# HpWang-whu/RoReg

Measured on AMD Instinct MI355X. Metric: pair-registrations/sec, higher is better.
Workload: dtype f32 (every f32 operand enters the fp16 matrix cores as hi + lo fp16 under a per-keypoint power-of-two block scale: <= 22 significant bits relative to a CONSERVATIVE per-keypoint bound -- measured on the extractor: the bound sits 2^2..2^6 above the keypoint's true coefficient maximum (config.f16x2_sc

## Files before the change

include/roreg_hip.h:

```cpp
#ifndef ROREG_HIP_H
#define ROREG_HIP_H

#include <stdint.h>
#include <stddef.h>

#ifdef __cplusplus
extern "C" {
#endif

#define ROREG_ABI_VERSION 6
int roreg_abi_version(void);
const char *roreg_last_error(void);

int roreg_set_group_tables(const int32_t *P_host, const int32_t *Nei_host, const double *R_host);

size_t roreg_group_conv_packed_size(int Cin, int Cout, int KS);
int roreg_group_conv_pack_weights(const float *W_host , int Cin, int Cout, int KS,
                                  float *wpack_host );
size_t roreg_group_conv_workspace_size(int B, int Cin, int Cout, int Lin, int Lout, int KS);
int roreg_group_conv(const float *x, const float *wpack, const float *bias,
                     const float *bn_scale, const float *bn_shift, const float *residual,
                     float *out, const int32_t *gather,
                     int B, int Cin, int Cout, int Lin, int Lout, int KS,
                     float *workspace, size_t workspace_floats, void *stream);
// ... 174 lines not shown
int roreg_context_colmax(const float *R, int L, const int32_t *seg_off, int n_seg, int max_len, float *ctx_out, float *ws, void *stream);

int roreg_knn_attention(const float *qp, const float *kp, const float *vp, const int64_t *idx, int k_is_table, int v_is_table,
                        int m, int k, float *x_out, void *stream);

int roreg_rm_elementwise(int op, const float *a, const float *b, const float *c, const int64_t *idx, int L, int k, int C,
                         float *out, float *ws, void *stream);

size_t roreg_sinkhorn_workspace_size(int m, int n);
int roreg_sinkhorn(const float *src_final, int m, const float *tgt_final, int n, float alpha, int iters, float *Z_out,
                   int64_t *matches0, int64_t *matches1, float *mscores0, float *mscores1, float *ws, size_t ws_floats, void *stream);

size_t roreg_sinkhorn_batch_workspace_size(int n_seg, int max_m, int max_n, long long total_m, long long total_n);
int roreg_sinkhorn_batch_consts(const int32_t *seg_src_host, const int32_t *seg_tgt_host, int n_seg, float *consts_host);
int roreg_sinkhorn_batch(const float *src_final, const float *tgt_final, const int32_t *seg_src, const int32_t *seg_tgt,
                         const int32_t *seg_src_host, const int32_t *seg_tgt_host, const float *consts, int n_seg, float alpha, int iters,
                         int64_t *matches0, int64_t *matches1, float *mscores0, float *mscores1, float *ws, size_t ws_floats,
                         void *stream);

size_t roreg_sinkhorn_batch2_workspace_size(int n_seg, int max_m, int max_n, long long total_m, long long total_n);
int roreg_sinkhorn_batch2(const float *src_final, const float *tgt_final, const int32_t *seg_src, const int32_t *seg_tgt,
                          const int32_t *seg_src_host, const int32_t *seg_tgt_host, const float *consts, int n_seg, float alpha, int iters,
                          int64_t *matches0, int64_t *matches1, float *mscores0, float *mscores1, float *ws, size_t ws_floats,
                          int recompute, void *stream);
size_t roreg_sinkhorn_batch3_workspace_size(int n_seg, int max_m, int max_n, long long total_m, long long total_n, int recompute, int want_Z);
int roreg_sinkhorn_batch3(const float *src_final, const float *tgt_final, const int32_t *seg_src, const int32_t *seg_tgt,
                          const int32_t *seg_src_host, const int32_t *seg_tgt_host, const float *consts, int n_seg, float alpha, int iters,
                          int64_t *matches0, int64_t *matches1, float *mscores0, float *mscores1, float *ws, size_t ws_floats,
                          int recompute, float *Z_out, void *stream);
int roreg_write_files(const char *const *paths, const void *const *headers, const int32_t *header_len, const void *const *data,
                      const int64_t *nbytes, int n, int n_threads);
int roreg_yohoc_draw_many(const uint32_t *seeds, int n_pairs, const int64_t *anchors, const int64_t *offsets, int max_iter, int max_tries,
                          int64_t *rows_out, int32_t *n_hyp_out, double *giveup_out, int n_threads);
size_t roreg_mlp_head_workspace(int L, int n_seg, int C1);
int roreg_mlp_head(const float *x, const float *pos, const float *table, const int64_t *idx, const float *conf, int m, int k, int L, int Cin,
                   const float *W1, const float *b1, int C1, const float *Wr, const float *br, float *h, float *y, const int32_t *seg_off,
                   int n_seg, int mult, float eps, float *mean_rstd, double *ws, void *stream);
int roreg_sinkhorn_early_exit(int on);
int roreg_sinkhorn_iteration_stats(long long *iterations, long long *pairs, int reset, void *stream);

int roreg_set_fourier_tables(const float *F_host);
size_t roreg_irrep_gemm_tiles(int O, int B, int32_t *tiles_host);
size_t roreg_irrep_gemm_tiles_m(int O, int B, int tile_m , int32_t *tiles_host);
int roreg_irrep_gemm(const float *const *X, float *const *Out, const float *const *Add, const float *const *Wpack, int C, int O, int B,
                     const int32_t *tiles_dev, int n_tiles, void *stream);
int roreg_irrep_gemm_split(const float *const *X, float *const *Out, const float *const *Add, const void *const *Wsplit, int C, int O, int B,
                           const int32_t *tiles_dev, int n_tiles, void *stream);
int roreg_irrep_gemm_f16x2(const float *const *X, float *const *Out, const float *const *Add, const void *const *Wsplit2,
                           const float *x_bound_dev, int w_exp, const float *next_u_dev, const float *next_v_dev, float *out_bound_dev,
                           int C, int O, int B, const int32_t *tiles_dev, int n_tiles,
                           int tile_m ,
                           int x_planes , void *stream);
int roreg_gemm_persistent(int on);
int roreg_row_bound(const void *x_spatial, int x_bf16 , const float *bn_scale, const float *bn_shift,
                    float *bound_out, int B, int C, void *stream);
int roreg_ft_nonlin(const float *Xin , const float *x_spatial, const float *bias,
                    const float *bias2, const float *bn_scale, const float *bn_shift, const float *resid_spatial,
                    float *Xout , float *out_spatial ,
                    const int32_t *g_map ,
                    int Lout , int Lvalid,
                    int B, int C, int split ,
                    const float *out_bound ,
                    float *out_rowmax ,
                    int spatial_bf16 ,
                    int out_planes ,
                    void *stream);
int roreg_ft_nonlin_packed(const float *Xin, const float *bias, const float *bn_scale, const float *bn_shift, uint32_t *out_words,
                           const int32_t *g_map, int Lout, int Lvalid, int B, int C, const float *out_bound, float *raw_col, int raw_g,
                           void *stream);
int roreg_ft_nonlin_gathered(const uint64_t *rows , const int64_t *dr , int feat_bf16, const float *bn_scale ,
                             const float *bn_shift, float *Xout, int B, const float *out_bound , int out_planes, void *stream);

typedef struct roreg_icp_grid_desc {
    double origin[3];
    double edge;
    int32_t dims[3];
    int32_t n;
    int64_t cells;
    int64_t reserved;
} roreg_icp_grid_desc;
size_t roreg_icp_grid_size(const double *lo_host, const double *hi_host, int n, double max_dist, roreg_icp_grid_desc *desc_host,
                           size_t *workspace_bytes);
int roreg_icp_grid_build(const float *points, const roreg_icp_grid_desc *desc_host, void *grid, void *workspace, size_t workspace_bytes,
                         void *stream);
typedef struct roreg_icp_task {
    const void *tgt_grid;
    const void *src_grid;
    const double *T0;
    int32_t n_src;
    int32_t slot0;
} roreg_icp_task;
size_t roreg_icp_batch_workspace(int n_tasks, long long total_slots);
int roreg_icp_batch(const roreg_icp_task *tasks, int n_tasks, const int32_t *work, int n_work, long long total_slots, double max_dist,
                    int max_iter, double tol_deg, double tol_t, double *T_out, int32_t *iters_out, int32_t *inliers_out, double *rmse_out,
                    int32_t *status_out, int32_t *assign_out, double *stats_out, void *workspace, size_t workspace_bytes, void *stream);

int roreg_icp_normals(const void *grid, double radius, int min_neighbors, double *out, void *stream);
typedef struct roreg_icp_plane_task {
    const void *tgt_grid;
    const void *src_grid;
    const double *tgt_normals;
    const double *T0;
    int32_t n_src;
    int32_t slot0;
} roreg_icp_plane_task;
size_t roreg_icp_plane_batch_workspace(int n_tasks, long long total_slots);
// ... 16 lines not shown
```

roreg_amd/_abi.py:

```python
import ctypes
from ctypes import c_int, c_void_p, c_size_t, c_double, c_float, c_char_p

import numpy as np

ABI_VERSION = 6

_P = c_void_p
PROTOTYPES = {
    'roreg_abi_version': (c_int, []),
    'roreg_last_error': (c_char_p, []),
    'roreg_set_group_tables': (c_int, [_P, _P, _P]),
    'roreg_group_conv_packed_size': (c_size_t, [c_int, c_int, c_int]),
    'roreg_group_conv_pack_weights': (c_int, [_P, c_int, c_int, c_int, _P]),
    'roreg_group_conv_workspace_size': (c_size_t, [c_int, c_int, c_int, c_int, c_int, c_int]),
    'roreg_group_conv': (c_int, [_P, _P, _P, _P, _P, _P, _P, _P, c_int, c_int, c_int, c_int, c_int, c_int, _P, c_size_t, _P]),
    'roreg_group_conv_split': (c_int, [_P, _P, _P, _P, _P, _P, _P, _P, c_int, c_int, c_int, c_int, c_int, c_int, c_int, _P]),
    'roreg_group_conv_f16x2': (c_int, [_P, _P, c_int, _P, _P, _P, c_float, c_float, _P, _P, _P, _P, _P, c_int, c_int, c_int, c_int, c_int, c_int, c_int, _P]),
    'roreg_group_conv_f16x2_packed': (c_int, [_P, _P, c_int, _P, _P, _P, _P, _P, _P, c_int, c_int, c_int, c_int, c_int, c_int, c_int, _P]),
    'roreg_dense_f16x2': (c_int, [_P, _P, c_int, _P, _P, _P, c_float, c_float, _P, _P, c_int, _P, _P, c_int, c_int, c_int, _P]),
    'roreg_dense_split': (c_int, [_P, _P, _P, _P, _P, _P, c_int, _P, c_int, c_int, c_int, _P]),
    'roreg_gf_finalize': (c_int, [_P, _P, c_int, _P, c_int, _P]),
    'roreg_det_score': (c_int, [_P, _P, c_int, _P]),
    'roreg_inv_descriptor': (c_int, [_P, c_int, _P, c_int, _P]),
    'roreg_nn_search': (c_int, [_P, _P, c_int, _P, _P, c_int, c_int, _P, _P, _P, _P]),
# ... 2 lines not shown
    'roreg_knn_search_workspace': (c_size_t, [c_int, c_int]),
    'roreg_knn_search': (c_int, [_P, c_int, _P, c_int, c_int, c_int, _P, _P, c_size_t, _P]),
    'roreg_knn_search_ex': (c_int, [_P, c_int, _P, c_int, c_int, c_int, c_int, _P, _P, _P, c_size_t, _P]),
    'roreg_knn_search_seg_workspace': (c_size_t, [ctypes.c_longlong, c_int, c_int, c_int]),
    'roreg_knn_search_seg': (c_int, [_P, _P, _P, _P, c_int, ctypes.c_longlong, c_int, c_int, c_int, c_int, _P, _P, c_size_t, _P]),
    'roreg_mutual_matches': (c_int, [_P, _P, c_int, c_int, _P, _P, _P, _P, _P]),
    'roreg_mutual_match_batch_workspace': (c_size_t, [c_int, c_int]),
    'roreg_mutual_match_batch': (c_int, [_P, c_int, c_int, _P, _P, _P, c_size_t, _P]),
    'roreg_des2r': (c_int, [_P, _P, _P, _P, c_int, _P, _P, _P]),
    'roreg_set_des2r_tables': (c_int, [c_int, _P, _P, _P, _P]),
    'roreg_group_corr_irrep': (c_int, [_P, _P, _P, _P, c_int, c_int, _P, _P]),
    'roreg_group_corr_mfma': (c_int, [_P, _P, _P, _P, c_int, c_int, _P, _P]),
    'roreg_des2r_irrep': (c_int, [_P, _P, _P, _P, _P, _P, c_int, c_int, _P, _P]),
    'roreg_des2r_recheck_count': (c_int, [c_int, _P]),
    'roreg_feat_coefs': (c_int, [_P, c_int, _P, c_int, c_int, c_int, _P]),
    'roreg_et_gather': (c_int, [_P, _P, _P, _P, c_int, _P, _P, _P, c_int, _P, _P]),
    'roreg_quat_to_trans': (c_int, [_P, _P, _P, _P, _P, _P, c_int, _P, _P, _P]),
    'roreg_ransac_score': (c_int, [_P, _P, _P, c_int, c_int, _P, _P, c_int, c_double, _P, _P, _P, _P]),
    'roreg_refine': (c_int, [_P, _P, _P, c_int, c_int, _P, c_int, _P, _P, _P, c_double, _P, _P, _P]),
    'roreg_lt_prepare_batch': (c_int, [_P, c_int, c_int, c_int, _P, _P, _P, _P, _P, _P]),
    'roreg_lt_finish_batch': (c_int, [_P, c_int, c_int, _P, _P, _P, _P]),
    'roreg_role_max': (c_int, [_P, _P, c_int, _P, _P, _P, c_int, _P]),
    'roreg_row_bound_roles': (c_int, [_P, c_int, _P, _P, _P, _P, c_int, _P]),
    'roreg_inv_descriptor_roles': (c_int, [_P, c_int, _P, _P, _P, _P, c_int, _P]),
    'roreg_lt_prepare_rows': (c_int, [_P, _P, c_int, c_int, c_int, _P, _P, _P, _P]),
    'roreg_ransac_batch_workspace': (c_size_t, [c_int, ctypes.c_longlong, c_int]),
    'roreg_ransac_batch': (c_int, [_P, c_int, ctypes.c_longlong, c_int, c_int, c_double, c_int, _P, _P, _P, _P, _P, _P, c_size_t, _P]),
    'roreg_refine_batch': (c_int, [_P, _P, c_int, ctypes.c_longlong, _P, ctypes.c_double, c_int, _P, _P, _P, _P]),
    'roreg_yohoc_draw': (c_int, [_P, ctypes.c_longlong, _P, _P, c_int, c_int, _P, _P, _P, _P]),
    'roreg_gather_rows_batch': (c_int, [_P, c_int, c_int, c_int, _P]),
    'roreg_gather_rows_f64': (c_int, [_P, _P, c_int, c_int, _P, _P]),
    'roreg_group_corr': (c_int, [_P, _P, _P, _P, c_int, c_int, _P, _P, _P]),
    'roreg_topk_dot_workspace_size': (c_size_t, [c_int, c_int, c_int]),
    'roreg_topk_dot': (c_int, [_P, c_int, _P, c_int, c_int, _P, _P, _P, c_size_t, _P, _P, c_int, c_int, c_int, _P]),
    'roreg_context_colmax': (c_int, [_P, c_int, _P, c_int, c_int, _P, _P, _P]),
    'roreg_sinkhorn_batch_workspace_size': (c_size_t, [c_int, c_int, c_int, ctypes.c_longlong, ctypes.c_longlong]),
    'roreg_sinkhorn_batch_consts': (c_int, [_P, _P, c_int, _P]),
    'roreg_sinkhorn_batch': (c_int, [_P, _P, _P, _P, _P, _P, _P, c_int, c_float, c_int, _P, _P, _P, _P, _P, c_size_t, _P]),
    'roreg_sinkhorn_batch2_workspace_size': (c_size_t, [c_int, c_int, c_int, ctypes.c_longlong, ctypes.c_longlong]),
    'roreg_sinkhorn_batch2': (c_int, [_P, _P, _P, _P, _P, _P, _P, c_int, c_float, c_int, _P, _P, _P, _P, _P, c_size_t, c_int, _P]),
    'roreg_sinkhorn_batch3_workspace_size': (c_size_t, [c_int, c_int, c_int, ctypes.c_longlong, ctypes.c_longlong, c_int, c_int]),
    'roreg_sinkhorn_batch3': (c_int, [_P, _P, _P, _P, _P, _P, _P, c_int, c_float, c_int, _P, _P, _P, _P, _P, c_size_t, c_int, _P, _P]),
    'roreg_write_files': (c_int, [_P, _P, _P, _P, _P, c_int, c_int]),
    'roreg_yohoc_draw_many': (c_int, [_P, c_int, _P, _P, c_int, c_int, _P, _P, _P, c_int]),
    'roreg_mlp_head_workspace': (c_size_t, [c_int, c_int, c_int]),
    'roreg_mlp_head': (c_int, [_P, _P, _P, _P, _P, c_int, c_int, c_int, c_int, _P, _P, c_int, _P, _P, _P, _P, _P, c_int, c_int, c_float, _P, _P, _P]),
    'roreg_sinkhorn_early_exit': (c_int, [c_int]),
    'roreg_sinkhorn_iteration_stats': (c_int, [_P, _P, c_int, _P]),
    'roreg_linear': (c_int, [_P, c_int, c_int, _P, _P, c_int, _P, _P]),
    'roreg_linear_mfma': (c_int, [_P, c_int, c_int, _P, _P, c_int, _P, _P]),
    'roreg_linear_path': (c_int, [c_int]),
    'roreg_linear_cat3': (c_int, [_P, _P, _P, _P, c_int, c_int, _P, _P, c_int, _P, _P]),
    'roreg_gemm_persistent': (c_int, [c_int]),
    'roreg_instnorm_stats': (c_int, [_P, c_int, c_int, c_float, _P, _P, _P, c_int, c_int, _P]),
    'roreg_mlp_tail': (c_int, [_P, c_int, c_int, _P, _P, _P, _P, _P, c_int, c_int, _P]),
    'roreg_mlp_tail_mfma': (c_int, [_P, c_int, c_int, _P, _P, _P, _P, _P, c_int, c_int, _P]),
    'roreg_knn_attention': (c_int, [_P, _P, _P, _P, c_int, c_int, c_int, c_int, _P, _P]),
    'roreg_rm_elementwise': (c_int, [c_int, _P, _P, _P, _P, c_int, c_int, c_int, _P, _P, _P]),
    'roreg_sinkhorn_workspace_size': (c_size_t, [c_int, c_int]),
    'roreg_sinkhorn': (c_int, [_P, c_int, _P, c_int, c_float, c_int, _P, _P, _P, _P, _P, _P, c_size_t, _P]),
    'roreg_icp_grid_size': (c_size_t, [_P, _P, c_int, c_double, _P, _P]),
    'roreg_icp_grid_build': (c_int, [_P, _P, _P, _P, c_size_t, _P]),
    'roreg_icp_batch_workspace': (c_size_t, [c_int, ctypes.c_longlong]),
    'roreg_icp_batch': (c_int, [_P, c_int, _P, c_int, ctypes.c_longlong, c_double, c_int, c_double, c_double, _P, _P, _P, _P, _P, _P, _P, _P, c_size_t, _P]),
    'roreg_icp_normals': (c_int, [_P, c_double, c_int, _P, _P]),
    'roreg_icp_plane_batch_workspace': (c_size_t, [c_int, ctypes.c_longlong]),
    'roreg_icp_plane_batch': (c_int, [_P, c_int, _P, c_int, ctypes.c_longlong, c_double, c_int, c_double, c_double, _P, _P, _P, _P, _P, _P, _P, _P, c_size_t, _P]),
    'roreg_voxel_workspace': (c_size_t, [c_int]),
    'roreg_voxel_downsample': (c_int, [_P, c_int, c_double, _P, _P, _P, _P, _P, _P, _P, c_size_t, _P]),
    'roreg_profile_enable': (c_int, [c_int]),
    'roreg_profile_read': (c_int, [c_int, _P, _P]),
    'roreg_set_fourier_tables': (c_int, [_P]),
    'roreg_mt_shuffle_prefix': (c_int, [_P, c_int, _P, c_int, c_int, _P, c_int]),
    'roreg_mt_stream_shuffle_prefix': (c_int, [_P, _P, _P, c_int, c_int, _P]),
    'roreg_irrep_gemm_tiles': (c_size_t, [c_int, c_int, _P]),
    'roreg_irrep_gemm_tiles_m': (c_size_t, [c_int, c_int, c_int, _P]),
    'roreg_irrep_gemm': (c_int, [_P, _P, _P, _P, c_int, c_int, c_int, _P, c_int, _P]),
    'roreg_irrep_gemm_split': (c_int, [_P, _P, _P, _P, c_int, c_int, c_int, _P, c_int, _P]),
    'roreg_irrep_gemm_f16x2': (c_int, [_P, _P, _P, _P, _P, c_int, _P, _P, _P, c_int, c_int, c_int, _P, c_int, c_int, c_int, _P]),
    'roreg_row_bound': (c_int, [_P, c_int, _P, _P, _P, c_int, c_int, _P]),
    'roreg_ft_nonlin': (c_int, [_P, _P, _P, _P, _P, _P, _P, _P, _P, _P, c_int, c_int, c_int, c_int, c_int, _P, _P, c_int, c_int, _P]),
    'roreg_ft_nonlin_packed': (c_int, [_P, _P, _P, _P, _P, _P, c_int, c_int, c_int, c_int, _P, _P, c_int, _P]),
    'roreg_ft_nonlin_gathered': (c_int, [_P, _P, c_int, _P, _P, _P, c_int, _P, c_int, _P]),
}


_RANSAC_TASK = np.dtype([('keys0', np.uint64), ('keys1', np.uint64), ('matches', np.uint64), ('w', np.uint64), ('Trans', np.uint64),
                         ('hyp_rows', np.uint64), ('M', np.int32), ('H', np.int32), ('koff', np.int64)])

_MATCH_TASK = np.dtype([('desc0', np.uint64), ('desc1', np.uint64), ('rows0', np.uint64), ('rows1', np.uint64), ('m0', np.int32), ('m1', np.int32)])

_GATHER_TASK = np.dtype([('src', np.uint64), ('rows', np.uint64), ('dst', np.uint64), ('n', np.int32), ('pad', np.int32)])

_LT_TASK = np.dtype([('before0', np.uint64), ('before1', np.uint64), ('after0', np.uint64), ('after1', np.uint64), ('keys0', np.uint64),
                     ('keys1', np.uint64), ('matches', np.uint64), ('sel', np.uint64), ('n', np.int32), ('pad', np.int32), ('off', np.int64),
                     ('coef0', np.uint64), ('coef1', np.uint64)])

_ICP_GRID_DESC = np.dtype([('origin', np.float64, 3), ('edge', np.float64), ('dims', np.int32, 3), ('n', np.int32), ('cells', np.int64),
                           ('reserved', np.int64)])

_ICP_TASK = np.dtype([('tgt_grid', np.uint64), ('src_grid', np.uint64), ('T0', np.uint64), ('n_src', np.int32), ('slot0', np.int32)])

_ICP_PLANE_TASK = np.dtype([('tgt_grid', np.uint64), ('src_grid', np.uint64), ('tgt_normals', np.uint64), ('T0', np.uint64), ('n_src', np.int32),
                            ('slot0', np.int32)])
```

roreg_amd/_hip_fourier.py:

```python
import os
from ctypes import c_void_p

import numpy as np
import torch

from . import hip as _core
from .hip import HipError, _check, _feat, _ptr, _stream, lib

__all__ = ['DenseSplitLayer', 'IRREP_DIMS', 'IRREP_OFFSETS', '_bf16_split3', '_keypoint_of_columns', '_ptr_array', '_res_ptr', '_tile_cache', 'bf16_split3_frags', 'bf16_split3_pack', 'bound_exp', 'coef_pitch', 'coef_size', 'coef_views', 'dense_split', 'ensure_fourier', 'f16_scale_exp', 'f16_split2_frags', 'f16_split2_pack', 'frag_pack', 'ft_nonlin', 'ft_nonlin_gathered', 'ft_nonlin_packed', 'gemm_persistent', 'group_conv_split_pack', 'irrep_gemm', 'next_bound', 'next_bound_spatial', 'pack_coefs_f16x2', 'row_bound', 'unpack_coefs_f16x2', 'words_to_planes']


_fourier_ready = False
IRREP_DIMS = (1, 3, 3, 4, 5)
IRREP_OFFSETS = (0, 1, 10, 19, 35, 60)


def ensure_fourier():
    global _fourier_ready
    if not _fourier_ready:
        from .fourier import group_fourier
        F = np.ascontiguousarray(group_fourier().F, np.float32)
        _check(lib().roreg_set_fourier_tables(F.ctypes.data), 'roreg_set_fourier_tables')
        _fourier_ready = True


def _ptr_array(views):
    arr = (c_void_p * 5)(*[c_void_p(v.data_ptr()) for v in views])
    return arr


def coef_pitch(B):
    return (int(B) + 31) // 32 * 32


def coef_size(C, B):
    return 60 * C * coef_pitch(B)


def coef_views(buf, C, B):
    Bp = coef_pitch(B)
    return [buf[IRREP_OFFSETS[r] * C * Bp:IRREP_OFFSETS[r + 1] * C * Bp].view(IRREP_DIMS[r] * C, IRREP_DIMS[r] * Bp) for r in range(5)]


_tile_cache = {}


def irrep_gemm(X_buf, Wpacks, C, O, B, split=None, add=None, f16x2=None, x_bound=None, next_bound=None, x_planes=False):
    Bp = coef_pitch(B)
    if X_buf.numel() != 60 * C * Bp or (add is not None and add.numel() != 60 * O * Bp):
        raise HipError(f'irrep_gemm: coefficient buffers must hold 60*C*{Bp} floats (B={B} padded to the 32-keypoint pitch)')
    out = torch.empty(60 * O * Bp, dtype=torch.float32, device=X_buf.device)
    tile_m = 256 if (f16x2 is not None and O % 256 == 0 and not os.environ.get('ROREG_TILE_M128')) else 128
    key = (O, Bp, tile_m)
    t = _tile_cache.get(key)
    if t is None:
        n = lib().roreg_irrep_gemm_tiles_m(O, Bp, tile_m, None)
        host = np.empty((n, 3), np.int32)
        lib().roreg_irrep_gemm_tiles_m(O, Bp, tile_m, host.ctypes.data)
        t = torch.from_numpy(host).cuda()
        _tile_cache[key] = t
    xv = coef_views(X_buf, C, B); ov = coef_views(out, O, B)
    av = _ptr_array(coef_views(add, O, B)) if add is not None else None
    if _core.PROFILE is not None:
        e0 = torch.cuda.Event(enable_timing=True); e1 = torch.cuda.Event(enable_timing=True); e0.record()
    bound_out = None
    if f16x2 is not None:
        wl, w_exp = f16x2
        if x_bound is None or x_bound.numel() != Bp:
            raise HipError(f'irrep_gemm: the fp16 x 2 GEMM needs x_bound with one value per (padded) keypoint ({Bp})')
        nu = nv = None
        if next_bound is not None:
            nu, nv = next_bound
            if nu.numel() != O or nv.numel() != O:
                raise HipError('irrep_gemm: next_bound must hold one (u, v) per output channel')
            bound_out = torch.zeros(Bp, dtype=torch.float32, device=X_buf.device)
        _check(lib().roreg_irrep_gemm_f16x2(_ptr_array(xv), _ptr_array(ov), av, _ptr_array(wl), _ptr(x_bound, torch.float32), int(w_exp),
                                            _ptr(nu, torch.float32), _ptr(nv, torch.float32), _ptr(bound_out), C, O, Bp,
                                            _ptr(t, torch.int32), int(t.shape[0]), tile_m, (int(x_planes) if x_planes in (1, 2) and x_planes is not True else (2 if _core.MFMA16 else 1)) if x_planes else 0, _stream()), 'roreg_irrep_gemm_f16x2')
    elif split is not None:
        _check(lib().roreg_irrep_gemm_split(_ptr_array(xv), _ptr_array(ov), av, _ptr_array(split), C, O, Bp, _ptr(t, torch.int32), int(t.shape[0]),
                                            _stream()), 'roreg_irrep_gemm_split')
    else:
        _check(lib().roreg_irrep_gemm(_ptr_array(xv), _ptr_array(ov), av, _ptr_array(Wpacks), C, O, Bp, _ptr(t, torch.int32), int(t.shape[0]), _stream()),
               'roreg_irrep_gemm')
    if _core.PROFILE is not None:
        e1.record(); _core.PROFILE.append((('irrep_gemm_f16x2' if f16x2 is not None else 'irrep_gemm_split' if split is not None else 'irrep_gemm', Bp, C, O), e0, e1))
    return (out, bound_out) if next_bound is not None else out


class gemm_persistent:

    def __init__(self, on=True):
        self.on = int(on)

    def __enter__(self):
        self.prev = lib().roreg_gemm_persistent(self.on)

    def __exit__(self, *exc):
        lib().roreg_gemm_persistent(self.prev)
        return False


def row_bound(x, bn=None, roles=None):
    B, C = int(x.shape[0]), int(x.shape[1])
    out = torch.empty(coef_pitch(B), dtype=torch.float32, device=x.device)
    scale, shift = bn if bn is not None else (None, None)
    xp, bf = _feat(x)
    if roles is not None:
        if bn is not None or C != 32:
            raise HipError('row_bound: roles go with the 32-channel input features and no BatchNorm')
        r_scale, r_shift, role = _core._role_args(roles, B)
        _check(lib().roreg_row_bound_roles(xp, bf, _ptr(out), _ptr(r_scale), _ptr(r_shift), _ptr(role), B, _stream()), 'roreg_row_bound_roles')
        return out
    _check(lib().roreg_row_bound(xp, bf, _ptr(scale), _ptr(shift), _ptr(out), B, C, _stream()), 'roreg_row_bound')
    return out


def _keypoint_of_columns(d, Bp):
    n = torch.arange(d * Bp, device='cuda')
    return ((n // 32) // d) * 32 + (n % 32)


def bound_exp(bound):
    _, ex = torch.frexp(bound.float())
    e = torch.where((bound > 0) & torch.isfinite(bound), 14 - ex, torch.zeros_like(ex))
    return e.clamp(-100, 100)


def pack_coefs_f16x2(X_buf, C, B, bound=None):
    Bp = coef_pitch(B)
    views = coef_views(X_buf, C, B)
    if bound is None:
        bound = torch.zeros(Bp, dtype=torch.float32, device=X_buf.device)
        for r, v in enumerate(views):
            kp = _keypoint_of_columns(IRREP_DIMS[r], Bp)
            bound.scatter_reduce_(0, kp, v.abs().amax(0), 'amax')
    e = bound_exp(bound)
    out = torch.empty_like(X_buf)
    for r, (v, o) in enumerate(zip(views, coef_views(out, C, B))):
        kp = _keypoint_of_columns(IRREP_DIMS[r], Bp)
        y = torch.ldexp(v, e[kp][None, :])
        hi = y.half()
        lo = (y - hi.float()).half()
        w = (hi.view(torch.int16).to(torch.int32) & 0xffff) | (lo.view(torch.int16).to(torch.int32) << 16)
        o.copy_(w.view(torch.float32))
    return out, bound


def words_to_planes(X_words, C, B):
    w = X_words.contiguous().view(torch.int32).view(-1, 2, 16)
    hi = (w & 0xffff).to(torch.int16).transpose(1, 2); lo = (w >> 16).to(torch.int16).transpose(1, 2)
    return torch.cat([hi.reshape(-1, 32), lo.reshape(-1, 32)], 1).contiguous().view(torch.float32).view(-1)


def unpack_coefs_f16x2(X_words, bound, C, B):
# ... 181 lines not shown
```

roreg_amd/csrc/fourier.hip:

```cpp
#include "common.h"
#include "primitives.h"
#include <algorithm>
#include <atomic>
#include <cmath>
#include <cstdlib>
#include <type_traits>
#include <utility>
#include <vector>

namespace {

constexpr int NIRR = 5;

struct GemmDescs {
    const float *X[NIRR];
    float *Out[NIRR];
    const float *Add[NIRR];
    const float4 *W[NIRR];
    int K[NIRR], M[NIRR], Mpad[NIRR], N[NIRR];
};

template <int CT>
__global__ __launch_bounds__(256, 2) void irrep_gemm_kernel(GemmDescs p, const int *__restrict__ tiles) {
    extern __shared__ __attribute__((aligned(16))) char smem[];
// ... 434 lines not shown
            };
            auto rb = [&](int t) { b[t][0] = xn[xslot[t]]; b[t][1] = xn[2 * NCOL + xslot[t]]; __builtin_amdgcn_sched_barrier(0); };
            auto ra = [&](int ot) { an[ot][0] = aq[ot * 32]; an[ot][1] = aq[2 * OT + ot * 32]; __builtin_amdgcn_sched_barrier(0); };
            __builtin_amdgcn_sched_barrier(0);
            mm(0, 0); dma(0); mm(0, 1); dma(1); mm(0, 2); rb(0);
            mm(1, 0); ra(0);  mm(1, 1); ra(1);  mm(1, 2); rb(1);
            mm(2, 0);
            ROREG_WAIT_X(2, xr_use);
            store_plane(xd, xr_use, 0, 0);
            if constexpr (CPT == 2) store_plane(xd, xr_use, 1, 0);
            __builtin_amdgcn_sched_barrier(0);
            mm(2, 1);
            store_plane(xd, xr_use, 0, 1);
            if constexpr (CPT == 2) store_plane(xd, xr_use, 1, 1);
            __builtin_amdgcn_sched_barrier(0);
            mm(2, 2); rb(2);
            mm(3, 0); ldx(0, 3); mm(3, 1); ldx(3, 6); mm(3, 2); ldx(6, 8); rb(3);
            asm volatile("s_waitcnt vmcnt(8) lgkmcnt(0)\n\ts_barrier" ::: "memory");
        };
        xword xa0[8], xa1[8];
        load_xa(0, xa0); issue_a(0, 0);
        load_xa(1, xa1); issue_a(1, 1);
        ROREG_WAIT_X(0, xa0);
        ROREG_WAIT_X(0, xa1);
        store_x(0, xa0);
        load_xa(2, xa0);
        store_x(1, xa1);
        asm volatile("s_waitcnt vmcnt(8) lgkmcnt(0)\n\ts_barrier" ::: "memory");
        read_a(0, aA);
#pragma unroll
        for (int t = 0; t < 4; ++t) read_b(0, t);
        asm volatile("s_waitcnt lgkmcnt(0)\n\ts_barrier" ::: "memory");
        for (int ks = 0; ks < nsteps; ks += 2) {
            step2(ks, 0, xa1, xa0, aA, aB);
            step2(ks + 1, 1, xa0, xa1, aB, aA);
        }
        asm volatile("s_waitcnt vmcnt(0)" ::: "memory");
#undef ROREG_WAIT_X
    } else {
        load_x(0, xr0);
        issue_a(0, 0);
        load_x(1, xr1);
        convert_store(0, xr0);
        asm volatile("s_waitcnt vmcnt(0)" ::: "memory");
        __syncthreads();
        for (int ks = 0; ks < nsteps; ks += 2) {
            step(ks, 0, xr0, xr1);
            step(ks + 1, 1, xr1, xr0);
        }
    }
    gemm_split_epilogue<NP, WO>(p, irr, mt, n0, wo, ncol_wave, acc, smem);
}


template <int BIG>
__global__ __launch_bounds__(512, 2) void irrep_gemm_xdma_kernel(GemmSplitDescs p, const int *__restrict__ tiles) {
    using frag = f16x8;
    extern __shared__ __attribute__((aligned(16))) char smem[];
    constexpr int NCOL = 256, OT = 256;
    constexpr int XIMG = 16 * NCOL * 2, XSTAGE = 2 * XIMG;
    constexpr int ABUF = 2 * 2 * OT;
    char *xs = smem;
    frag *as = reinterpret_cast<frag *>(smem + 3 * XSTAGE);
    const int tid = threadIdx.x, lane = tid & 63, w = tid >> 6;
    const int j = lane & 31, h = lane >> 5;
    const int irr = tiles[blockIdx.x * 3], mt = tiles[blockIdx.x * 3 + 1], nt = tiles[blockIdx.x * 3 + 2];
    if (irr < 0) return;
    const frag *__restrict__ W = reinterpret_cast<const frag *>(p.W[irr]);
    const int K = p.K[irr], Mpad = p.Mpad[irr], N = p.N[irr];
    const size_t split_stride = (size_t)(K / 16) * 2 * Mpad;
    const int wo = w % 4, wb = w / 4;
    const int n0 = nt * NCOL;
    const int ncol_wave = wb * 128;
    const int nsteps = K / 16;

    f32x16 acc[2][4];
#pragma unroll
    for (int a = 0; a < 2; ++a)
#pragma unroll
        for (int t = 0; t < 4; ++t)
#pragma unroll
            for (int r = 0; r < 16; ++r) acc[a][t][r] = 0.f;

    const int x_plane = w >> 2;
    const char *xsrc[2];
    int xdst[2];
#pragma unroll
    for (int i2 = 0; i2 < 2; ++i2) {
        const int mm = (2 * w + i2) & 7;
        const int pi = mm * 64 + lane;
        const int beta = pi >> 3, r = (pi & 7) >> 1, half = pi & 1;
        const int k = 4 * (beta >> 4) + r;
        int col = n0 + 16 * (beta & 15) + 8 * half;
        if (col > N - 8) col = N - 8;
        xsrc[i2] = reinterpret_cast<const char *>(p.X[irr]) + (size_t)k * N * 4 + (col >> 5) * 128 + x_plane * 64 + (col & 31) * 2;
        xdst[i2] = x_plane * XIMG + mm * 1024;
    }
    const size_t xstep = (size_t)16 * N * 4;
    auto dma_x = [&](int i2, int kstep, int stage) {
        const char *q = xsrc[i2] + (size_t)(kstep < nsteps ? kstep : nsteps - 1) * xstep;
        __builtin_amdgcn_global_load_lds((const __attribute__((address_space(1))) void *)q,
                                         (__attribute__((address_space(3))) void *)(xs + stage * XSTAGE + xdst[i2]), 16, 0, 0);
    };
    const frag *wsrc = W + (size_t)(tid / OT) * Mpad + mt * OT + (tid % OT);
    auto dma_w = [&](int sp, int kstep, int buf) {
        const frag *q = wsrc + (size_t)(kstep < nsteps ? kstep : nsteps - 1) * 2 * Mpad;
// ... 1360 lines not shown
                stream[k].push_back(bk.r); stream[k].push_back(mt); stream[k].push_back(nt);
            }
    }
    size_t longest = 0;
    for (int k = 0; k < 8; ++k) longest = std::max(longest, stream[k].size() / 3);
    const size_t n = longest * 8;
    if (tiles_host)
        for (size_t i = 0; i < longest; ++i)
            for (int k = 0; k < 8; ++k) {
                int32_t *t = tiles_host + (i * 8 + k) * 3;
                if (i * 3 < stream[k].size()) { t[0] = stream[k][i * 3]; t[1] = stream[k][i * 3 + 1]; t[2] = stream[k][i * 3 + 2]; }
                else { t[0] = -1; t[1] = 0; t[2] = 0; }
            }
    return n;
}

extern "C" int roreg_irrep_gemm(const float *const *X, float *const *Out, const float *const *Add, const float *const *Wpack, int C, int O, int B,
                                const int32_t *tiles_dev, int n_tiles, void *stream) {
    ROREG_REQUIRE(X && Out && Wpack && tiles_dev && C > 0 && O > 0 && B > 0 && n_tiles > 0, "roreg_irrep_gemm: bad arguments");
    ROREG_REQUIRE(C % 32 == 0, "roreg_irrep_gemm: C must be a multiple of 32 (got %d)", C);
    ROREG_REQUIRE(B % 4 == 0, "roreg_irrep_gemm: B must be a multiple of 4 (got %d); pad the keypoint batch", B);
    static const int dims[5] = {1, 3, 3, 4, 5};
    GemmDescs p;
    for (int r = 0; r < 5; ++r) {
        p.X[r] = X[r]; p.Out[r] = Out[r]; p.Add[r] = Add ? Add[r] : nullptr; p.W[r] = reinterpret_cast<const float4 *>(Wpack[r]);
        p.K[r] = dims[r] * C; p.M[r] = dims[r] * O; p.Mpad[r] = round_up(dims[r] * O, 128); p.N[r] = dims[r] * B;
    }
    constexpr int CT = 32;
    const size_t lds = 2 * CT * 256 * sizeof(float);
    auto kern = irrep_gemm_kernel<CT>;
    hipError_t e = hipFuncSetAttribute(reinterpret_cast<const void *>(kern), hipFuncAttributeMaxDynamicSharedMemorySize, (int)lds);
    if (e != hipSuccess) { roreg::set_error("roreg_irrep_gemm: hipFuncSetAttribute: %s", hipGetErrorString(e)); return 1; }
    hipLaunchKernelGGL(kern, dim3(n_tiles), dim3(256), lds, roreg::as_stream(stream), p, tiles_dev);
    ROREG_CHECK_LAUNCH("roreg_irrep_gemm");
    return 0;
}

#define ROREG_GEMM_PERSIST_DEFAULT 0
static std::atomic<int> g_gemm_persist{-1};
static int gemm_launch_form() {
    int v = g_gemm_persist.load(std::memory_order_relaxed);
    if (v < 0) {
        const char *e = getenv("ROREG_GEMM_PERSIST");
        v = e ? (e[0] == '1' ? 1 : e[0] == '2' ? 2 : 0) : ROREG_GEMM_PERSIST_DEFAULT;
        g_gemm_persist.store(v, std::memory_order_relaxed);
    }
    return v;
}
extern "C" int roreg_gemm_persistent(int on) {
    const int prev = gemm_launch_form();
    if (on >= 0 && on <= 2) g_gemm_persist.store(on, std::memory_order_relaxed);
    return prev;
}
static int gemm_cu_count() {
    static const int n = [] {
        int dev = 0, cus = 0;
        if (hipGetDevice(&dev) != hipSuccess || hipDeviceGetAttribute(&cus, hipDeviceAttributeMultiprocessorCount, dev) != hipSuccess || cus <= 0) cus = 256;
        return cus;
    }();
    return n;
}
template <int NP, int WO>
static int launch_gemm_split(const char *what, const float *const *X, float *const *Out, const float *const *Add, const void *const *Wsplit,
                             const float *xbound, int w_exp, const float *nb_u, const float *nb_v, float *out_bound, int C, int O, int B,
                             const int32_t *tiles_dev, int n_tiles, void *stream, int x_planes = 0) {
    static const int dims[5] = {1, 3, 3, 4, 5};
    GemmSplitDescs p;
    for (int r = 0; r < 5; ++r) {
        p.X[r] = X[r]; p.Out[r] = Out[r]; p.Add[r] = Add ? Add[r] : nullptr; p.W[r] = Wsplit[r];
        p.K[r] = dims[r] * C; p.M[r] = dims[r] * O; p.Mpad[r] = round_up(dims[r] * O, 128); p.N[r] = dims[r] * B;
        if (WO == 4 && p.Mpad[r] % 256 != 0) { roreg::set_error("%s: tile_m = 256 needs O %% 256 == 0 (got %d)", what, O); return 2; }
    }
    p.xbound = xbound; p.w_exp = w_exp; p.nb_u = nb_u; p.nb_v = nb_v; p.out_bound = out_bound; p.O = O;
    constexpr int CT = 32;
    const size_t lds = 2 * (NP * 2 * 256 + NP * (WO * 64) * 2) * 16;
    if (x_planes) {
        if constexpr (NP == 2 && WO == 4) {
            const size_t lds_x = 3 * (2 * 16 * 256 * 2) + 2 * (2 * 2 * 256) * 16;
            const bool mfma16 = x_planes == 2;
            const size_t lds_use = mfma16 ? (size_t)(6 + 4) * 16384 : lds_x;
            auto kx = mfma16 ? ((long long)C * O == 256ll * 512 ? irrep_gemm_xdma16_kernel<1> : irrep_gemm_xdma16_kernel<0>)
                             : ((long long)C * O == 256ll * 512 ? irrep_gemm_xdma_kernel<1> : irrep_gemm_xdma_kernel<0>);
            hipError_t e = hipFuncSetAttribute(reinterpret_cast<const void *>(kx), hipFuncAttributeMaxDynamicSharedMemorySize, (int)lds_use);
            if (e != hipSuccess) { roreg::set_error("%s: hipFuncSetAttribute: %s", what, hipGetErrorString(e)); return 1; }
            if (mfma16 && gemm_launch_form() == 2) {
                auto kh = (long long)C * O == 256ll * 512 ? irrep_gemm_xdma16h_kernel<1> : irrep_gemm_xdma16h_kernel<0>;
                const size_t lds_h = (size_t)6 * 8192 + 2 * 16384;
                e = hipFuncSetAttribute(reinterpret_cast<const void *>(kh), hipFuncAttributeMaxDynamicSharedMemorySize, (int)lds_h);
                if (e != hipSuccess) { roreg::set_error("%s: hipFuncSetAttribute: %s", what, hipGetErrorString(e)); return 1; }
                hipLaunchKernelGGL(kh, dim3(2 * n_tiles), dim3(256), lds_h, roreg::as_stream(stream), p, tiles_dev);
            } else if (mfma16 && gemm_launch_form() == 1) {
                const bool big = (long long)C * O == 256ll * 512;
                static const int ra = [] { const char *v = getenv("ROREG_GEMM_PERSIST_RA"); return v ? atoi(v) : 2; }();
                auto kp = ra == 0 ? (big ? irrep_gemm_xdma16p_kernel<1, 0> : irrep_gemm_xdma16p_kernel<0, 0>)
                        : ra == 4 ? (big ? irrep_gemm_xdma16p_kernel<1, 4> : irrep_gemm_xdma16p_kernel<0, 4>)
                                  : (big ? irrep_gemm_xdma16p_kernel<1, 2> : irrep_gemm_xdma16p_kernel<0, 2>);
                e = hipFuncSetAttribute(reinterpret_cast<const void *>(kp), hipFuncAttributeMaxDynamicSharedMemorySize, (int)lds_use);
                if (e != hipSuccess) { roreg::set_error("%s: hipFuncSetAttribute: %s", what, hipGetErrorString(e)); return 1; }
                const int wgs = std::min(n_tiles, std::max(8, gemm_cu_count() / 8 * 8));
                hipLaunchKernelGGL(kp, dim3(wgs), dim3(512), lds_use, roreg::as_stream(stream), p, tiles_dev, n_tiles / 8);
            } else {
                hipLaunchKernelGGL(kx, dim3(n_tiles), dim3(512), lds_use, roreg::as_stream(stream), p, tiles_dev);
            }
            hipError_t e2 = hipGetLastError();
            if (e2 != hipSuccess) { roreg::set_error("%s: launch failed: %s", what, hipGetErrorString(e2)); return 1; }
            return 0;
        } else {
            roreg::set_error("%s: the half-block layout needs the fp16 x 2 kernel with tile_m = 256", what);
            return 2;
        }
    }
    static const int pipe = [] { const char *e = getenv("ROREG_GEMM_PIPE"); return e ? atoi(e) : 1; }();
    auto kern = (long long)C * O == 256ll * 512 ? irrep_gemm_split_kernel<CT, NP, WO, 1> : irrep_gemm_split_kernel<CT, NP, WO, 0>;
    if constexpr (NP == 2) { if (pipe == 1) kern = (long long)C * O == 256ll * 512 ? irrep_gemm_split_kernel<CT, NP, WO, 1, 1> : irrep_gemm_split_kernel<CT, NP, WO, 0, 1>; }
    hipError_t e = hipFuncSetAttribute(reinterpret_cast<const void *>(kern), hipFuncAttributeMaxDynamicSharedMemorySize, (int)lds);
    if (e != hipSuccess) { roreg::set_error("%s: hipFuncSetAttribute: %s", what, hipGetErrorString(e)); return 1; }
    hipLaunchKernelGGL(kern, dim3(n_tiles), dim3(WO * 128), lds, roreg::as_stream(stream), p, tiles_dev);
    hipError_t e2 = hipGetLastError();
    if (e2 != hipSuccess) { roreg::set_error("%s: launch failed: %s", what, hipGetErrorString(e2)); return 1; }
    return 0;
}

extern "C" int roreg_irrep_gemm_split(const float *const *X, float *const *Out, const float *const *Add, const void *const *Wsplit, int C, int O, int B,
                                      const int32_t *tiles_dev, int n_tiles, void *stream) {
    ROREG_REQUIRE(X && Out && Wsplit && tiles_dev && C > 0 && O > 0 && B > 0 && n_tiles > 0, "roreg_irrep_gemm_split: bad arguments");
    ROREG_REQUIRE(C % 32 == 0 && B % 4 == 0, "roreg_irrep_gemm_split: C %% 32 and B %% 4 must be 0 (got %d, %d)", C, B);
// ... 209 lines not shown
```

Measured before the change: 1111.

## Add specialized thin-K and thin-M irrep GEMM kernels for 32-wide shapes

Adds two new f16x2 split irrep GEMM kernels, dispatched by default when C==32 (thin K) or O==32 (thin M) with no Add or x_planes. The thin-K kernel keeps the whole X fragment in registers and streams weight blocks into LDS with double-buffered async DMA, overlapping output stores and bound computation with the next block's MFMAs. The thin-M kernel keeps all output rows in registers and triple-buffers weight and X loads across K steps. Both aim to replace the general 256-tile path, which wastes work and occupancy on these skinny shapes. The cost is substantial hand-scheduled code with manual waitcnt counts, which is fragile.

```diff
diff --git a/include/roreg_hip.h b/include/roreg_hip.h
--- a/include/roreg_hip.h
+++ b/include/roreg_hip.h
@@ -250,6 +250,7 @@
                            int tile_m ,
                            int x_planes , void *stream);
 int roreg_gemm_persistent(int on);
+int roreg_gemm_thin(int on);
 int roreg_row_bound(const void *x_spatial, int x_bf16 , const float *bn_scale, const float *bn_shift,
                     float *bound_out, int B, int C, void *stream);
 int roreg_ft_nonlin(const float *Xin , const float *x_spatial, const float *bias,
diff --git a/roreg_amd/_abi.py b/roreg_amd/_abi.py
--- a/roreg_amd/_abi.py
+++ b/roreg_amd/_abi.py
@@ -78,6 +78,7 @@
     'roreg_linear_path': (c_int, [c_int]),
     'roreg_linear_cat3': (c_int, [_P, _P, _P, _P, c_int, c_int, _P, _P, c_int, _P, _P]),
     'roreg_gemm_persistent': (c_int, [c_int]),
+    'roreg_gemm_thin': (c_int, [c_int]),
     'roreg_instnorm_stats': (c_int, [_P, c_int, c_int, c_float, _P, _P, _P, c_int, c_int, _P]),
     'roreg_mlp_tail': (c_int, [_P, c_int, c_int, _P, _P, _P, _P, _P, c_int, c_int, _P]),
     'roreg_mlp_tail_mfma': (c_int, [_P, c_int, c_int, _P, _P, _P, _P, _P, c_int, c_int, _P]),
diff --git a/roreg_amd/_hip_fourier.py b/roreg_amd/_hip_fourier.py
--- a/roreg_amd/_hip_fourier.py
+++ b/roreg_amd/_hip_fourier.py
@@ -7,7 +7,7 @@
 from . import hip as _core
 from .hip import HipError, _check, _feat, _ptr, _stream, lib
 
-__all__ = ['DenseSplitLayer', 'IRREP_DIMS', 'IRREP_OFFSETS', '_bf16_split3', '_keypoint_of_columns', '_ptr_array', '_res_ptr', '_tile_cache', 'bf16_split3_frags', 'bf16_split3_pack', 'bound_exp', 'coef_pitch', 'coef_size', 'coef_views', 'dense_split', 'ensure_fourier', 'f16_scale_exp', 'f16_split2_frags', 'f16_split2_pack', 'frag_pack', 'ft_nonlin', 'ft_nonlin_gathered', 'ft_nonlin_packed', 'gemm_persistent', 'group_conv_split_pack', 'irrep_gemm', 'next_bound', 'next_bound_spatial', 'pack_coefs_f16x2', 'row_bound', 'unpack_coefs_f16x2', 'words_to_planes']
+__all__ = ['DenseSplitLayer', 'IRREP_DIMS', 'IRREP_OFFSETS', '_bf16_split3', '_keypoint_of_columns', '_ptr_array', '_res_ptr', '_tile_cache', 'bf16_split3_frags', 'bf16_split3_pack', 'bound_exp', 'coef_pitch', 'coef_size', 'coef_views', 'dense_split', 'ensure_fourier', 'f16_scale_exp', 'f16_split2_frags', 'f16_split2_pack', 'frag_pack', 'ft_nonlin', 'ft_nonlin_gathered', 'ft_nonlin_packed', 'gemm_persistent', 'gemm_thin', 'group_conv_split_pack', 'irrep_gemm', 'next_bound', 'next_bound_spatial', 'pack_coefs_f16x2', 'row_bound', 'unpack_coefs_f16x2', 'words_to_planes']
 
 
 _fourier_ready = False
@@ -101,6 +101,19 @@
         return False
 
 
+class gemm_thin:
+
+    def __init__(self, on=True):
+        self.on = int(bool(on))
+
+    def __enter__(self):
+        self.prev = lib().roreg_gemm_thin(self.on)
+
+    def __exit__(self, *exc):
+        lib().roreg_gemm_thin(self.prev)
+        return False
+
+
 def row_bound(x, bn=None, roles=None):
     B, C = int(x.shape[0]), int(x.shape[1])
     out = torch.empty(coef_pitch(B), dtype=torch.float32, device=x.device)
diff --git a/roreg_amd/csrc/fourier.hip b/roreg_amd/csrc/fourier.hip
--- a/roreg_amd/csrc/fourier.hip
+++ b/roreg_amd/csrc/fourier.hip
@@ -510,6 +510,330 @@
     gemm_split_epilogue<NP, WO>(p, irr, mt, n0, wo, ncol_wave, acc, smem);
 }
 
+typedef float f32x4 __attribute__((ext_vector_type(4)));
+__device__ __forceinline__ f16x8 lds_frag_read(unsigned addr, int off) {
+    f16x8 v;
+    asm volatile("ds_read_b128 %0, %1 offset:%2" : "=v"(v) : "v"(addr), "i"(off));
+    return v;
+}
+#define ROREG_WAIT_LDS2(a, b) asm volatile("s_waitcnt lgkmcnt(0)" : "+v"(a), "+v"(b))
+template <bool THIN_M>
+__device__ __host__ __forceinline__ int thin_tile_cols(int irr) { return THIN_M && irr >= 3 ? 128 : 256; }
+template <bool THIN_M>
+__device__ __forceinline__ void thin_wg_irrep(const GemmSplitDescs &p, int &irr, int &nt) {
+    int wg = blockIdx.x;
+    irr = NIRR - 1;
+    for (; irr > 0; --irr) {
+        const int tc = thin_tile_cols<THIN_M>(irr), nts = (p.N[irr] + tc - 1) / tc;
+        if (wg < nts) break;
+        wg -= nts;
+    }
+    nt = wg;
+}
+__device__ __forceinline__ void words_to_frags(const unsigned (&v)[8], f16x8 &hi, f16x8 &lo) {
+    u32x4 H, L;
+#pragma unroll
+    for (int i = 0; i < 4; ++i) {
+        H[i] = __builtin_amdgcn_perm(v[2 * i + 1], v[2 * i], 0x05040100u);
+        L[i] = __builtin_amdgcn_perm(v[2 * i + 1], v[2 * i], 0x07060302u);
+    }
+    hi = __builtin_bit_cast(f16x8, H); lo = __builtin_bit_cast(f16x8, L);
+}
+
+template <int D>
+__device__ __forceinline__ void thin_k_body(const GemmSplitDescs &p, int irr, int nt, f16x8 *as, float *uv ) {
+    constexpr int NS = 2 * D;
+    constexpr int NI = 2 * NS;
+    constexpr int NDMA = (NI + 7) / 8;
+    constexpr int SLOT = NI * 64;
+    const int tid = threadIdx.x, lane = tid & 63, w = tid >> 6, j = lane & 31, h = lane >> 5;
+    const int N = p.N[irr], Mpad = p.Mpad[irr], O = p.O;
+    const int nblk = D * O / 32;
+    const f16x8 *__restrict__ W = reinterpret_cast<const f16x8 *>(p.W[irr]);
+    const size_t split_stride = (size_t)NS * 2 * Mpad;
+    const int n = nt * 256 + w * 32 + j;
+    const bool live = n < N;
+    const int nl = live ? n : N - 32 + j;
+
+    const f16x8 *wsrc[NDMA];
+    int wdst[NDMA];
+#pragma unroll
+    for (int q = 0; q < NDMA; ++q) {
+        const int i = (w + 8 * q) % NI, sp = i / NS, ks = i % NS;
+        wsrc[q] = W + sp * split_stride + (size_t)(ks * 2 + h) * Mpad + j;
+        wdst[q] = i * 64;
+    }
+    auto dma = [&](int blk, int slot) {
+#pragma unroll
+        for (int q = 0; q < NDMA; ++q)
+            __builtin_amdgcn_global_load_lds((const __attribute__((address_space(1))) void *)(wsrc[q] + blk * 32),
+                                             (__attribute__((address_space(3))) void *)(as + slot * SLOT + wdst[q]), 16, 0, 0);
+        __builtin_amdgcn_sched_barrier(0);
+        asm volatile("" ::: "memory");
+    };
+    dma(0, 0);
+
+    f16x8 bh[NS], bl[NS];
+    {
+        const unsigned *xq = reinterpret_cast<const unsigned *>(p.X[irr]) + nl + (size_t)(8 * h) * N;
+#pragma unroll
+        for (int s = 0; s < NS; ++s) {
+            unsigned v[8];
+#pragma unroll
+            for (int e = 0; e < 8; ++e) v[e] = __builtin_nontemporal_load(xq + (size_t)(16 * s + e) * N);
+            words_to_frags(v, bh[s], bl[s]);
+        }
+    }
+    if (!live) {
+        for (int blk = 0; blk < nblk; ++blk) {
+            asm volatile("s_waitcnt vmcnt(0) lgkmcnt(0)\n\ts_barrier" ::: "memory");
+            dma(blk + 1 < nblk ? blk + 1 : nblk - 1, (blk + 1) & 1);
+        }
+        asm volatile("s_waitcnt vmcnt(0)" ::: "memory");
+        return;
+    }
+    const float oscale = ldexpf(1.f, -(bound_exp(p.xbound[column_keypoint(n, D)]) + p.w_exp));
+    float bmax = 0.f;
+    float *__restrict__ Out = p.Out[irr];
+    const unsigned ocol = (unsigned)(4 * h) * (unsigned)N + (unsigned)n;
+    const unsigned uvbase = (unsigned)(uintptr_t)uv + 16 * h;
+
+    auto store_quad = [&](int pb, const f32x16 &c, int rq, const f32x4 &u, const f32x4 &v, auto bound_c) {
+        float *ob = Out + (size_t)(pb * 32 + 8 * rq) * N;
+        #pragma unroll
+        for (int rr = 0; rr < 4; ++rr) {
+            const float o = c[rq * 4 + rr] * oscale;
+            __builtin_nontemporal_store(o, ob + (size_t)rr * N + ocol);
+            if constexpr (decltype(bound_c)::value) bmax = fmaxf(bmax, fmaf(u[rr], fabsf(o), v[rr]));
+        }
+    };
+    auto read_uv = [&](int pb, int rq, f32x4 &u, f32x4 &v) {
+        const unsigned a = uvbase + (unsigned)(((pb * 32) % O + 8 * rq) * 4);
+        asm volatile("ds_read_b128 %0, %1" : "=v"(u) : "v"(a));
+        asm volatile("ds_read_b128 %0, %1" : "=v"(v) : "v"(a + 4 * 512));
+    };
+    auto block = [&](int blk, f32x16 &cur, const f32x16 &prev, auto drain_c, auto w16_c, auto bound_c) {
+        constexpr bool DRAIN = decltype(drain_c)::value, BOUND = decltype(bound_c)::value;
+        if constexpr (decltype(w16_c)::value) asm volatile("s_waitcnt vmcnt(16)\n\ts_barrier" ::: "memory");
+        else asm volatile("s_waitcnt vmcnt(0) lgkmcnt(0)\n\ts_barrier" ::: "memory");
+        dma(blk + 1 < nblk ? blk + 1 : nblk - 1, (blk + 1) & 1);
+        const unsigned abase = (unsigned)(uintptr_t)(as + (blk & 1) * SLOT) + lane * 16;
+        f16x8 a[2][2];
+        a[0][0] = lds_frag_read(abase, 0); a[0][1] = lds_frag_read(abase, NS * 1024);
+#pragma unroll
+        for (int r = 0; r < 16; ++r) cur[r] = 0.f;
+#pragma unroll
+        for (int s = 0; s < NS; ++s) {
+            f32x4 u[4], v[4];
+#pragma unroll
+            for (int rq = 0; rq < 4; ++rq)
+                if (DRAIN && BOUND && rq * NS / 4 == s) read_uv(blk - 1, rq, u[rq], v[rq]);
+            ROREG_WAIT_LDS2(a[s & 1][0], a[s & 1][1]);
+#pragma unroll
+            for (int rq = 0; rq < 4; ++rq)
+                if (DRAIN && BOUND && rq * NS / 4 == s) ROREG_WAIT_LDS2(u[rq], v[rq]);
+            if (s + 1 < NS) { a[(s + 1) & 1][0] = lds_frag_read(abase, (s + 1) * 1024); a[(s + 1) & 1][1] = lds_frag_read(abase, (NS + s + 1) * 1024); }
+            cur = __builtin_amdgcn_mfma_f32_32x32x16_f16(a[s & 1][1], bh[s], cur, 0, 0, 0);
+            cur = __builtin_amdgcn_mfma_f32_32x32x16_f16(a[s & 1][0], bl[s], cur, 0, 0, 0);
+            cur = __builtin_amdgcn_mfma_f32_32x32x16_f16(a[s & 1][0], bh[s], cur, 0, 0, 0);
+#pragma unroll
+            for (int rq = 0; rq < 4; ++rq)
+                if (DRAIN && rq * NS / 4 == s) store_quad(blk - 1, prev, rq, u[rq], v[rq], bound_c);
+        }
+    };
+    auto run = [&](auto bound_c) {
+        using T = std::true_type; using F = std::false_type;
+        f32x16 c0, c1;
+#pragma unroll
+        for (int r = 0; r < 16; ++r) { c0[r] = 0.f; c1[r] = 0.f; }
+        block(0, c0, c1, F{}, F{}, bound_c);
+        if (nblk > 1) block(1, c1, c0, T{}, F{}, bound_c);
+        for (int blk = 2; blk < nblk; blk += 2) {
+            block(blk, c0, c1, T{}, T{}, bound_c);
+            if (blk + 1 < nblk) block(blk + 1, c1, c0, T{}, T{}, bound_c);
+        }
+        const f32x16 &last = (nblk & 1) ? c0 : c1;
+        f32x4 u[4], v[4];
+        if constexpr (decltype(bound_c)::value) {
+#pragma unroll
+            for (int rq = 0; rq < 4; ++rq) read_uv(nblk - 1, rq, u[rq], v[rq]);
+#pragma unroll
+            for (int rq = 0; rq < 4; ++rq) ROREG_WAIT_LDS2(u[rq], v[rq]);
+        }
+#pragma unroll
+        for (int rq = 0; rq < 4; ++rq) store_quad(nblk - 1, last, rq, u[rq], v[rq], bound_c);
+    };
+    if (p.out_bound != nullptr) {
+        run(std::true_type{});
+        const float bm = fmaxf(bmax, __shfl_xor(bmax, 32));
+        if (h == 0) atomicMax(reinterpret_cast<unsigned *>(p.out_bound) + column_keypoint(n, D), __float_as_uint(bm));
+    } else {
+        run(std::false_type{});
+    }
+    asm volatile("s_waitcnt vmcnt(0)" ::: "memory");
+}
+
+__global__ __launch_bounds__(512) void irrep_gemm_thin_k_kernel(GemmSplitDescs p) {
+    __shared__ __attribute__((aligned(16))) f16x8 as[2 * 20 * 64];
+    __shared__ __attribute__((aligned(16))) float uv[2 * 512];
+    if (p.out_bound != nullptr)
+        for (int i = threadIdx.x; i < p.O; i += 512) { uv[i] = p.nb_u[i]; uv[512 + i] = p.nb_v[i]; }
+    int irr, nt;
+    thin_wg_irrep<false>(p, irr, nt);
+    switch (irr) {
+        case 0: thin_k_body<1>(p, irr, nt, as, uv); break;
+        case 1: case 2: thin_k_body<3>(p, irr, nt, as, uv); break;
+        case 3: thin_k_body<4>(p, irr, nt, as, uv); break;
+        default: thin_k_body<5>(p, irr, nt, as, uv); break;
+    }
+}
+
+template <int D, int CB>
+__device__ __forceinline__ void thin_m_body(const GemmSplitDescs &p, int irr, int nt, f16x8 *as) {
+    constexpr int NI = 2 * D;
+    constexpr int NDMA = (NI + 3) / 4;
+    constexpr int SLOT = NI * 64;
+    const int tid = threadIdx.x, lane = tid & 63, w = tid >> 6, j = lane & 31, h = lane >> 5;
+    const int N = p.N[irr], Mpad = p.Mpad[irr], K = p.K[irr];
+    const int nsteps = K / 16;
+    const f16x8 *__restrict__ W = reinterpret_cast<const f16x8 *>(p.W[irr]);
+    const size_t split_stride = (size_t)nsteps * 2 * Mpad;
+    const int n = nt * (128 * CB) + w * (32 * CB) + CB * j;
+    const bool live = n < N;
+    const int nl = live ? n : N - CB;
+
+    const f16x8 *wsrc[NDMA];
+    int wdst[NDMA];
+#pragma unroll
+    for (int q = 0; q < NDMA; ++q) {
+        const int i = (w + 4 * q) % NI, sp = i / D, rb = i % D;
+        wsrc[q] = W + sp * split_stride + (size_t)h * Mpad + rb * 32 + j;
+        wdst[q] = i * 64;
+    }
+    auto dma = [&](int s, int slot) {
+        const size_t off = (size_t)(s < nsteps ? s : nsteps - 1) * 2 * Mpad;
+#pragma unroll
+        for (int q = 0; q < NDMA; ++q)
+            __builtin_amdgcn_global_load_lds((const __attribute__((address_space(1))) void *)(wsrc[q] + off),
+                                             (__attribute__((address_space(3))) void *)(as + slot * SLOT + wdst[q]), 16, 0, 0);
+        __builtin_amdgcn_sched_barrier(0);
+    };
+    const unsigned *xp = reinterpret_cast<const unsigned *>(p.X[irr]);
+    const unsigned xoff = ((unsigned)(8 * h) * (unsigned)N + (unsigned)nl) * 4u;
+    typedef typename std::conditional<CB == 1, unsigned, unsigned long long>::type xword;
+    auto load_x = [&](int s, xword (&x)[8]) {
+        const unsigned *q = xp + (size_t)(s < nsteps ? s : nsteps - 1) * 16 * N;
+#pragma unroll
+        for (int e = 0; e < 8; ++e) {
+            if constexpr (CB == 1) asm volatile("global_load_dword %0, %1, %2" : "=v"(x[e]) : "v"(xoff), "s"(q + (size_t)e * N) : "memory");
+            else asm volatile("global_load_dwordx2 %0, %1, %2" : "=v"(x[e]) : "v"(xoff), "s"(q + (size_t)e * N) : "memory");
+        }
+        __builtin_amdgcn_sched_barrier(0);
+    };
+#define ROREG_WAIT_X(cnt, xr) asm volatile("s_waitcnt vmcnt(" #cnt ")" : "+v"(xr[0]), "+v"(xr[1]), "+v"(xr[2]), "+v"(xr[3]), "+v"(xr[4]), "+v"(xr[5]), "+v"(xr[6]), "+v"(xr[7]) :: "memory")
+
+    f32x16 acc[D][CB];
+#pragma unroll
+    for (int rb = 0; rb < D; ++rb)
+#pragma unroll
+        for (int cb = 0; cb < CB; ++cb)
+#pragma unroll
+            for (int r = 0; r < 16; ++r) acc[rb][cb][r] = 0.f;
+
+    auto step = [&](int s, int slot, xword (&x)[8]) {
+        if constexpr (NDMA == 1) ROREG_WAIT_X(9, x); else if constexpr (NDMA == 2) ROREG_WAIT_X(10, x); else ROREG_WAIT_X(11, x);
+        asm volatile("s_barrier" ::: "memory");
+        f16x8 bh[CB], bl[CB];
+#pragma unroll
+        for (int cb = 0; cb < CB; ++cb) {
+            unsigned v[8];
+#pragma unroll
+            for (int e = 0; e < 8; ++e) v[e] = (unsigned)(x[e] >> (CB == 1 ? 0 : 32 * cb));
+            words_to_frags(v, bh[cb], bl[cb]);
+        }
+        __builtin_amdgcn_sched_barrier(0);
+        const int fill = slot >= 1 ? slot - 1 : 2;
+        dma(s + 2, fill);
+        load_x(s + 2, x);
+        const unsigned abase = (unsigned)(uintptr_t)(as + slot * SLOT) + lane * 16;
+        f16x8 a[2][2];
+        a[0][0] = lds_frag_read(abase, 0); a[0][1] = lds_frag_read(abase, D * 1024);
+#pragma unroll
+        for (int rb = 0; rb < D; ++rb) {
+            ROREG_WAIT_LDS2(a[rb & 1][0], a[rb & 1][1]);
+            if (rb + 1 < D) { a[(rb + 1) & 1][0] = lds_frag_read(abase, (rb + 1) * 1024); a[(rb + 1) & 1][1] = lds_frag_read(abase, (D + rb + 1) * 1024); }
+#pragma unroll
+            for (int cb = 0; cb < CB; ++cb) {
+                f32x16 c = acc[rb][cb];
+                c = __builtin_amdgcn_mfma_f32_32x32x16_f16(a[rb & 1][1], bh[cb], c, 0, 0, 0);
+                c = __builtin_amdgcn_mfma_f32_32x32x16_f16(a[rb & 1][0], bl[cb], c, 0, 0, 0);
+                c = __builtin_amdgcn_mfma_f32_32x32x16_f16(a[rb & 1][0], bh[cb], c, 0, 0, 0);
+                acc[rb][cb] = c;
+            }
+        }
+    };
+    xword xa[8], xb[8];
+    dma(0, 0); load_x(0, xa);
+    dma(1, 1); load_x(1, xb);
+    int slot = 0;
+    for (int s = 0; s < nsteps; s += 2) {
+        step(s, slot, xa);
+        slot = slot == 2 ? 0 : slot + 1;
+        step(s + 1, slot, xb);
+        slot = slot == 2 ? 0 : slot + 1;
+    }
+    ROREG_WAIT_X(0, xa);
+    ROREG_WAIT_X(0, xb);
+#undef ROREG_WAIT_X
+
+    if (!live) return;
+    float oscale[CB];
+#pragma unroll
+    for (int cb = 0; cb < CB; ++cb) oscale[cb] = ldexpf(1.f, -(bound_exp(p.xbound[column_keypoint(n + cb, D)]) + p.w_exp));
+    const bool want_bound = p.out_bound != nullptr;
+    float ur[16], vr[16], bmax[CB];
+#pragma unroll
+    for (int cb = 0; cb < CB; ++cb) bmax[cb] = 0.f;
+    if (want_bound) {
+#pragma unroll
+        for (int r = 0; r < 16; ++r) { const int o = (r & 3) + 8 * (r >> 2) + 4 * h; ur[r] = p.nb_u[o]; vr[r] = p.nb_v[o]; }
+    }
+    float *__restrict__ ob = p.Out[irr] + n + (size_t)(4 * h) * N;
+#pragma unroll
+    for (int rb = 0; rb < D; ++rb)
+#pragma unroll
+        for (int r = 0; r < 16; ++r) {
+            float o[CB];
+#pragma unroll
+            for (int cb = 0; cb < CB; ++cb) {
+                o[cb] = acc[rb][cb][r] * oscale[cb];
+                if (want_bound) bmax[cb] = fmaxf(bmax[cb], fmaf(ur[r], fabsf(o[cb]), vr[r]));
+            }
+            float *dst = ob + (size_t)(rb * 32 + (r & 3) + 8 * (r >> 2)) * N;
+            if constexpr (CB == 1) *dst = o[0]; else *reinterpret_cast<float2 *>(dst) = make_float2(o[0], o[CB - 1]);
+        }
+    if (want_bound) {
+#pragma unroll
+        for (int cb = 0; cb < CB; ++cb) {
+            const float bm = fmaxf(bmax[cb], __shfl_xor(bmax[cb], 32));
+            if (h == 0) atomicMax(reinterpret_cast<unsigned *>(p.out_bound) + column_keypoint(n + cb, D), __float_as_uint(bm));
+        }
+    }
+}
+
+__global__ __launch_bounds__(256, 2) void irrep_gemm_thin_m_kernel(GemmSplitDescs p) {
+    __shared__ __attribute__((aligned(16))) f16x8 as[3 * 10 * 64];
+    int irr, nt;
+    thin_wg_irrep<true>(p, irr, nt);
+    switch (irr) {
+        case 0: thin_m_body<1, 2>(p, irr, nt, as); break;
+        case 1: case 2: thin_m_body<3, 2>(p, irr, nt, as); break;
+        case 3: thin_m_body<4, 1>(p, irr, nt, as); break;
+        default: thin_m_body<5, 1>(p, irr, nt, as); break;
+    }
+}
+#undef ROREG_WAIT_LDS2
+
 
 template <int BIG>
 __global__ __launch_bounds__(512, 2) void irrep_gemm_xdma_kernel(GemmSplitDescs p, const int *__restrict__ tiles) {
@@ -1976,6 +2300,21 @@
     if (on >= 0 && on <= 2) g_gemm_persist.store(on, std::memory_order_relaxed);
     return prev;
 }
+static std::atomic<int> g_gemm_thin{-1};
+static int gemm_thin_on() {
+    int v = g_gemm_thin.load(std::memory_order_relaxed);
+    if (v < 0) {
+        const char *e = getenv("ROREG_GEMM_THIN");
+        v = e && e[0] == '0' ? 0 : 1;
+        g_gemm_thin.store(v, std::memory_order_relaxed);
+    }
+    return v;
+}
+extern "C" int roreg_gemm_thin(int on) {
+    const int prev = gemm_thin_on();
+    if (on == 0 || on == 1) g_gemm_thin.store(on, std::memory_order_relaxed);
+    return prev;
+}
 static int gemm_cu_count() {
     static const int n = [] {
         int dev = 0, cus = 0;
@@ -1996,6 +2335,17 @@
         if (WO == 4 && p.Mpad[r] % 256 != 0) { roreg::set_error("%s: tile_m = 256 needs O %% 256 == 0 (got %d)", what, O); return 2; }
     }
     p.xbound = xbound; p.w_exp = w_exp; p.nb_u = nb_u; p.nb_v = nb_v; p.out_bound = out_bound; p.O = O;
+    if constexpr (NP == 2) {
+        if (!x_planes && !Add && (O == 32 || (C == 32 && O % 32 == 0 && O <= 512)) && gemm_thin_on()) {
+            int wgs = 0;
+            for (int r = 0; r < 5; ++r) { const int tc = C == 32 ? thin_tile_cols<false>(r) : thin_tile_cols<true>(r); wgs += (p.N[r] + tc - 1) / tc; }
+            if (C == 32) hipLaunchKernelGGL(irrep_gemm_thin_k_kernel, dim3(wgs), dim3(512), 0, roreg::as_stream(stream), p);
+            else hipLaunchKernelGGL(irrep_gemm_thin_m_kernel, dim3(wgs), dim3(256), 0, roreg::as_stream(stream), p);
+            hipError_t e2 = hipGetLastError();
+            if (e2 != hipSuccess) { roreg::set_error("%s: launch failed: %s", what, hipGetErrorString(e2)); return 1; }
+            return 0;
+        }
+    }
     constexpr int CT = 32;
     const size_t lds = 2 * (NP * 2 * 256 + NP * (WO * 64) * 2) * 16;
     if (x_planes) {
```

Result: faster. 1126, median of 6 (+1.3%).
